# cts198859/deeprl_network

Hardware: AMD Instinct MI355X
Metric: env-steps/sec (agents x envs x steps/s), full rollout + A2C update loop (higher is better)
Workload: dtype f32; 1 GPU; CACC catchup, 8 agents x 4096 replicas/GPU, ia2c_fp (config_ia2c_fp_catchup.ini), n_step 60; replicas_per_gpu=4096, global_replicas=4096, parallelism=dp1, hipgraph_rollout=True, hipgraph_update=True, gemm_autotune=True

## Files before the change

deeprl_network_amd/_lib.py:

```python
import ctypes as C
import os

import torch

_PKG = os.path.dirname(os.path.abspath(__file__))
LIB_PATH = os.path.join(_PKG, 'libnmarl_hip.so')

if not os.path.exists(LIB_PATH):
    raise ImportError(
        'deeprl_network_amd: %s not found. Build it with `python -m deeprl_network_amd.build` '
        '(hipcc --offload-arch=gfx950). There is no CPU fallback.' % LIB_PATH)

from . import build as _build

if _build.built_hash() != _build.source_hash():
    raise ImportError(
        'deeprl_network_amd: %s is stale (built from sources %s, current sources %s). Rebuild it with '
        '`python -m deeprl_network_amd.build`.' % (LIB_PATH, _build.built_hash(), _build.source_hash()))

LIB_PATH = os.environ.get('NMARL_LIB_AB') or LIB_PATH
lib = C.CDLL(LIB_PATH)

ABI_VERSION = 4

# ... 179 lines not shown
    'nmarl_lstm_bptt_dial': [C.POINTER(BpttDial), _p],
    'nmarl_fc_fwd': [_i64, _i32, _i32, _i32, _p, _i64, _i64, _p, _i64, _p, _i64, _i32, _p, _i64, _i64, _p],
    'nmarl_fc_fwd_multi': [_i64, _i32, _i32, C.POINTER(FcPart), _i32, _p, _i64, _i64, _p],
    'nmarl_dial_msg_adjoint': [_i64, _i32, _i32, _p, _i64, _p, _i64, _p, _i64, _p, _i64, _p, _i64, _p, _i64, _p, _p, _p, _i32,
                               _p, _i64, _p, _i64, _p, _i64, _p, _i64, _p, _i64, _p],
    'nmarl_dial_msg_adjoint_parts': [_i64],
    'nmarl_onehot_argmax_add': [_i64, _i32, _i32, _i32, _p, _i64, _p, _p, _i64, _i64, _p],
    'nmarl_fc_bwd_chunks': [_i64, _i32],
    'nmarl_fc_bwd': [_i64, _i32, _i32, _i32, _p, _i64, _i64, _p, _i64, _i64, _p, _i64, _i64, _i32, _p, _p, _i64, _p, _i64, _p],
    'nmarl_fc_bwd_pair': [_i64, _i32, _p, _p, _i64, _i64, _p, _i64, _p, _i64, _i64, _i32, _p, _p, _p],
    'nmarl_fc_bwd_gather': [_i64, _i32, _i32, _i32, _p, _i32, _p, _i64, _i64, _p, _i64, _i64, _p, _i64, _i64, _i32, _p, _p, _i64, _p, _i64, _p],
    'nmarl_heads_loss': [_i64, _i32, _i32, _i32, _p, _i64, _p, _i64, _p, _i64, _p, _p, _p, _p, _f32, _f32, _p, _p, _p, _p, _p, _i64, _p, _i64, _p,
                         _i64, _p],
    'nmarl_thin_linear_bwd': [_i64, _i32, _i32, _i32, _p, _i64, _p, _i64, _p, _i64, _p, _i64, _p, _p, _i64, _p, _i64, _p, _i64, _p],
    'nmarl_nbr_action_value_fwd': [_i64, _i32, _i32, _i32, _p, _p, _p, _i64, _p, _i32, _p],
    'nmarl_nbr_action_value_bwd': [_i64, _i32, _i32, _i32, _p, _p, _p, _p, _p, _i64, _p],
    'nmarl_bias_act': [_i64, _i32, _i32, _p, _i64, _p, _i64, _i32, _p, _i64, _i64, _p],
    'nmarl_lstm_cell_bwd': [_i64, _i32, _i32, _p, _i64, _p, _i64, _p, _i64, _p, _p, _i64, _p, _i64, _p, _i64, _p, _i64, _p, _i64, _p],
    'nmarl_a2c_loss_chunks': [_i64, _i32],
    'nmarl_a2c_loss_fwd': [_i64, _i32, _i32, _p, _i64, _i64, _p, _p, _p, _p, _f32, _f32, _p, _p, _p],
    'nmarl_a2c_loss_bwd': [_i64, _i32, _i32, _p, _i64, _i64, _p, _p, _p, _p, _f32, _f32, _p, _p, _p, _p],
    'nmarl_sample_actions': [_i64, _i32, _i32, _p, _p, _i32, _u64, _i64, _i64, _p, _p, _p],
    'nmarl_nstep_return': [_i64, _i32, _i32, _p, _p, _p, _p, C.c_double, C.c_double, _p, _p, _p, _p],
    'nmarl_rmsprop_tf_clip': [_i32, _i64, _p, _p, _p, _p, _p, _f32, _f32, _f32, _f32, _f32, _p, _p],
    'nmarl_rmsprop_tf_clip_guarded': [_i32, _i64, _p, _p, _p, _p, _p, _f32, _f32, _f32, _f32, _f32, _p, _p, _p],
    'nmarl_handoff_capacity': [_i32, _i32],
    'nmarl_test_handoff_fault': [_i32],
    'nmarl_batch_epilogue': [C.POINTER(BatchEpilogue), _p],
    'nmarl_timestamp': [_p, _p],
    'nmarl_timestamp_rate_khz': [],
    'nmarl_copy_multi': [_i32, C.POINTER(_p), C.POINTER(_p), C.POINTER(_i64), _p, _p],
}

for _name, _args in SIGNATURES.items():
    _fn = getattr(lib, _name)
    _fn.argtypes = _args
    _fn.restype = C.c_int

if lib.nmarl_abi_version() != ABI_VERSION:
    raise ImportError('libnmarl_hip.so ABI %d != binding ABI %d: rebuild' %
                      (lib.nmarl_abi_version(), ABI_VERSION))


class NmarlError(RuntimeError):
    pass

# ... 24 lines not shown
```

deeprl_network_amd/agents/models.py:

```python
import logging
import os

import numpy as np
import torch

from .. import ops
from .policies import (ConsensusPolicy, DIALMultiAgentPolicy, FPPolicy, IC3MultiAgentPolicy, LstmPolicy,
                       NCMultiAgentPolicy)
from .utils import Scheduler

F32 = torch.float32


class IA2C:

    policy_cls = LstmPolicy
    per_agent_optimizer = True
    uses_fingerprint = False

    def __init__(self, n_s_ls, n_a_ls, neighbor_mask, distance_mask, coop_gamma, total_step, model_config,
                 seed=0, num_envs=1, device='cuda', dist_group=None, n_feat=None, n_feat_ls=None, obs_order=None):
        self.name = getattr(self, 'name', 'ia2c')
        self._init_algo(n_s_ls, n_a_ls, neighbor_mask, distance_mask, coop_gamma, total_step, seed,
                        model_config, num_envs, device, dist_group, n_feat, n_feat_ls, obs_order)
# ... 250 lines not shown
                os.environ.get('NMARL_MSG_CARRY', '1') == '0':
            return None
        if self._carry_buf is None:
            self._carry_buf = torch.zeros(self.n_agent, self.E, self.n_lstm, dtype=F32, device=self.device)
        d = dict(carry_in=self._carry_buf if (t > 0 and self._carry_holds == t) else None,
                 carry_out=self._carry_buf if t < self.n_step else None)
        mm = getattr(p, '_extra_full', {}).get('MM')
        if mm is not None and t + 1 < self.n_step and p.msg_kind == ops.MSG_MEAN_ADD:
            d['mean_next'] = mm[:, t + 1]
        self._carry_holds = t + 1 if t < self.n_step else -1
        return d

    S_bits = None

    def _relu_bits(self, t):
        if os.environ.get('NMARL_FC_BWD_PAIR', '1') == '0' or not getattr(self.policy, 'enc_writes_bits', False):
            return None
        if self.S_bits is None:
            self.S_bits = torch.zeros(self.n_agent, self.n_step, self.E, 4, dtype=torch.int32, device=self.device)
        p = self.policy
        p._bits_steps = 1 if t == 0 else p._bits_steps + 1
        return self.S_bits[:, t]

    def record(self, reward, done_post):
        t = self.t
        self.buf_r[t].copy_(self._norm_reward(reward))
        self.buf_done_post[t].copy_(done_post)
        self.t = t + 1

    def _norm_reward(self, r):
        if self.reward_norm > 0:
            r = r / self.reward_norm
        if self.reward_clip > 0:
            r = torch.clamp(r, -self.reward_clip, self.reward_clip)
        return r

    def load_rewards(self, raw_rewards):
        if self.reward_norm > 0:
            torch.div(raw_rewards, self.reward_norm, out=self.buf_r)
        else:
            torch.mul(raw_rewards, 1.0, out=self.buf_r)
        if self.reward_clip > 0:
            self.buf_r.clamp_(-self.reward_clip, self.reward_clip)
        self.t = self.n_step

    def bootstrap(self, done, action_scratch, mode=ops.SAMPLE_PHILOX, u=None, seed=0, env_id_base=0,
                  step=0, step_dev=None, done_is_zero=False, pre_encoded=False):
        assert self.t == self.n_step
        p = self.policy
        ob = None
        if pre_encoded:
            enc = self.encode_target(self.n_step)
        elif self.save_acts and p.enc_in_kernel(self.E, self.compact_obs):
            enc, ob = (self.encode_target(self.n_step) if p.coupled else None), dict(x=self.buf_x[self.n_step], fp=self.fp)
        elif self.save_acts and p.encodes_in_step(self.E, self.compact_obs):
            enc, ob = self.encode_target(self.n_step), self.buf_x[self.n_step]
        else:
            enc = p.encode(self.buf_x[self.n_step], self.fp)
        if self.save_acts and p.pv_one_launch(self.E):
            T = self.n_step
# ... 61 lines not shown
        per_agent = policy_loss + value_loss + entropy_loss
        self.last_loss = (policy_loss.detach(), value_loss.detach(), entropy_loss.detach(), per_agent.detach())
        return per_agent.sum()

    def update(self, R_end, rotate=True):
        lr = self.update_begin()
        self.update_grads(R_end)
        self.update_reduce()
        self.update_apply(lr, rotate=rotate)
        self.update_end()

    def update_begin(self):
        assert self.t == self.n_step, 'update() needs a full n_step batch (got %d)' % self.t
        self.cur_lr = self.lr_scheduler.get(self.n_step)
        return self.cur_lr

    @property
    def handoff_guarded(self):
        return bool(self.policy.coupled) and self.device.type == 'cuda'

    def update_grads(self, R_end):
        alpha = self.coop_gamma if self.coop_gamma >= 0 else -1.0
        T = self.n_step
        if self.save_acts and self.policy.pv_one_launch(self.E):
            with torch.no_grad():
                vn = self.buf_vn.view(self.n_agent, T * self.E)
                ops.nbr_action_value(self.buf_act.view(T * self.E, self.n_agent), self.policy.nbr_idx,
                                     self.policy.params['v_w'][:, self.n_lstm:], self.n_a, out=vn, accumulate=True)
                self.buf_v.copy_(self.buf_vn.permute(1, 0, 2))
        ops.nstep_return(self.buf_r, self.buf_v, self.buf_done_post, R_end.contiguous(), self.gamma, alpha,
                         self.dist_dev, self.R, self.Adv)
        ps = self.policy.params
        ps.begin_backward()
        FP = self.buf_fp[:T].permute(1, 0, 2, 3).reshape(self.n_agent, T * self.E, self.n_a)
        X = self.buf_x[:T]
        if self.save_acts:
            kw = {}
            if self.S_bits is not None and self.policy._bits_steps == T:
                kw['S_bits'] = self.S_bits
            Hs = self.policy.unroll_saved(X, FP, self.S_buf, self.G_buf, self.H_all, self.C_all,
                                          self.buf_done_pre, masked_steps=self.masked_steps, S_ext=self.S_ext, **kw)
        else:
            Hs = self.policy.unroll(X, FP, self.buf_done_pre, self.h_bw, self.c_bw, masked_steps=self.masked_steps)
        if not self._loss_backward_fused(Hs):
            loss = self._loss(Hs)
            loss.backward()
        ps.end_backward()
        if ps.mask is not None:
            ps.grad.mul_(ps.mask)
        if self._status_on_wire:
            ps.grad_tail.copy_(ops.handoff_status(self.device)[:1])

    @property
    def _status_on_wire(self):
# ... 14 lines not shown
            st = ops.handoff_status(self.device)[:1]
            torch.maximum(st, (ps.grad_tail != 0).to(torch.int32), out=st)
        if self.per_agent_optimizer:
            ops.rmsprop_tf_clip(ps.flat, ps.grad, ps.ms, ps.scratch, lr, self.rmsp_alpha, self.rmsp_epsilon,
                                self.max_grad_norm, scale, self.grad_norm, lr_dev=lr_dev, guard=guard)
        else:
            n = self.n_agent * ps.P
            ops.rmsprop_tf_clip(ps.flat.view(1, n), ps.grad.view(1, n), ps.ms.view(1, n), ps.scratch, lr,
                                self.rmsp_alpha, self.rmsp_epsilon, self.max_grad_norm, scale, self.grad_norm,
                                lr_dev=lr_dev, guard=guard)
        self._after_apply()
        if rotate:
            T = self.n_step
            self.h_bw.copy_(self.h_fw)
            self.c_bw.copy_(self.c_fw)
            self.buf_x[0].copy_(self.buf_x[T])
            self.buf_fp[0].copy_(self.buf_fp[T])

    def _after_apply(self):
        """Hook behind the optimiser step (ConseNet: the consensus averaging)."""

    def update_end(self):
        self.t = 0
        self.policy._enc_was_saved = False
        self.policy._bits_steps = 0
        self.policy._mm_was_saved = False

    def _obs_to_slab(self, obs):
        p = self.policy
        F, A = self.n_feat, self.n_a
        slab = np.zeros((1, self.n_agent, p.n_obs), dtype=np.float32)
        fp = None
        if not self._is_ma2c() and self.uses_fingerprint_obs():
            fp = np.zeros((self.n_agent, 1, p.n_na), dtype=np.float32)
        for i in range(self.n_agent):
            o = np.asarray(obs[i], dtype=np.float32)
            slab[0, i, :p.n_own[i]] = o[:p.n_own[i]]
            if self._is_ma2c():
                continue
            pos = p.n_own[i]
            for j in p.obs_order[i]:
                k = p.nbrs[i].index(j)
                slab[0, i, (k + 1) * F:(k + 1) * F + p.n_own[j]] = o[pos:pos + p.n_own[j]]
                pos += p.n_own[j]
            if fp is not None:
                for j in p.obs_order[i]:
# ... 176 lines not shown
```

deeprl_network_amd/csrc/a2c.hip:

```cpp
#include "common.h"

namespace {

__device__ __forceinline__ float sigmoidf_(float x) { return 1.0f / (1.0f + expf(-x)); }

struct CellStrides { int64_t z, z2, bias, c_prev, gates, c_new, h_new, dh, dh2, dc, dz, dc_prev; };

__global__ __launch_bounds__(256) void lstm_cell_fwd_kernel(
    const int64_t E, const int N, const int H, const CellStrides st, const float* __restrict__ z,
    const float* __restrict__ z2, const float* __restrict__ bias, const float* __restrict__ c_prev,
    const float* __restrict__ done, float* __restrict__ gates, float* __restrict__ c_new,
    float* __restrict__ h_new) {
    const int H4 = H >> 2;
    const int64_t total = (int64_t)N * E * H4;
    for (int64_t idx = (int64_t)blockIdx.x * blockDim.x + threadIdx.x; idx < total; idx += (int64_t)gridDim.x * blockDim.x) {
        const int64_t row = idx / H4;
        const int j = (int)(idx - row * H4) * 4;
        const int64_t n = row / E;
        const int64_t e = row - n * E;
        const float* zr = z + n * st.z + e * 4 * H;
        const float* b = bias + n * st.bias;
        float4 zi = *reinterpret_cast<const float4*>(zr + j), zf = *reinterpret_cast<const float4*>(zr + H + j);
        float4 zo = *reinterpret_cast<const float4*>(zr + 2 * H + j), zu = *reinterpret_cast<const float4*>(zr + 3 * H + j);
        if (z2 != nullptr) {
// ... 104 lines not shown
        } else {
            float uu;
            if (mode == 0) {
                uu = u[idx];
            } else {
                const Philox4 r = philox4x32_10((uint32_t)(env_id_base + e), (uint32_t)(n >> 2), (uint32_t)step,
                                                NMARL_STREAM_ACTION, (uint32_t)seed, (uint32_t)(seed >> 32));
                const uint32_t w = (n & 3) == 0 ? r.x : (n & 3) == 1 ? r.y : (n & 3) == 2 ? r.z : r.w;
                uu = u01_from_bits(w);
            }
            double tot = 0.0;
            for (int k = 0; k < A; ++k) tot += (double)p[k];
            double cum = 0.0;
            for (int k = 0; k < A; ++k) {
                cum += (double)p[k];
                if (cum / tot <= (double)uu) a = k + 1;
            }
            if (a > A - 1) a = A - 1;
        }
        action[idx] = (uint8_t)a;
    }
}

__global__ __launch_bounds__(256) void nstep_kernel(
    const int64_t E, const int N, const int T, const float* __restrict__ r, const float* __restrict__ v,
    const uint8_t* __restrict__ done_post, const float* __restrict__ R_end, const double gamma,
    const double alpha, const int32_t* __restrict__ dist, float* __restrict__ R_out, float* __restrict__ adv_out) {
    __shared__ double s_w[64 * 64];
    const bool spatial = alpha >= 0.0;
    if (spatial) {
        for (int p = threadIdx.x; p < N * N; p += blockDim.x) s_w[p] = dist[p] < 0 ? 0.0 : pow(alpha, (double)dist[p]);
        __syncthreads();
    }
    const int64_t total = (int64_t)N * E;
    for (int64_t idx = (int64_t)blockIdx.x * blockDim.x + threadIdx.x; idx < total; idx += (int64_t)gridDim.x * blockDim.x) {
        const int n = (int)(idx / E);
        const int64_t e = idx - (int64_t)n * E;
        double R = (double)R_end[idx];
        if (!spatial) {
            constexpr int U = 10;
            for (int t0 = T - 1; t0 >= 0; t0 -= U) {
                float rr[U], vv[U];
                uint8_t dd[U];
#pragma unroll
                for (int k = 0; k < U; ++k) {
                    const int t = t0 - k >= 0 ? t0 - k : 0;
                    dd[k] = done_post[(int64_t)t * E + e];
                    rr[k] = r[(int64_t)t * E + e];
                    vv[k] = v[((int64_t)t * N + n) * E + e];
                }
#pragma unroll
                for (int k = 0; k < U; ++k) {
                    const int t = t0 - k;
                    if (t < 0) break;
                    R = (double)rr[k] + gamma * R * (1.0 - (double)dd[k]);
                    const int64_t o = ((int64_t)n * T + t) * E + e;
                    R_out[o] = (float)R;
                    adv_out[o] = (float)(R - (double)vv[k]);
                }
            }
            continue;
        }
        for (int t = T - 1; t >= 0; --t) {
            const double keep = 1.0 - (double)done_post[(int64_t)t * E + e];
            if (!spatial) {
                R = (double)r[(int64_t)t * E + e] + gamma * R * keep;
            } else {
                R = gamma * R * keep;
                const float* rt = r + ((int64_t)t * E + e) * N;
                double add = 0.0;
                for (int j = 0; j < N; ++j) add += s_w[n * N + j] * (double)rt[j];
                R += add;
            }
            const int64_t o = ((int64_t)n * T + t) * E + e;
            R_out[o] = (float)R;
            adv_out[o] = (float)(R - (double)v[((int64_t)t * N + n) * E + e]);
        }
    }
}

struct EpilogueArgs {
    int64_t E;
    int32_t N, H, A, F, T, T_env;
    const float* g;
    const uint8_t* done;
    double *ep_sum, *ep_sq, *ep_len, *fin;
    float *h_fw, *c_fw, *h_bw, *c_bw;
    const float *fp_T, *fp_uniform, *x_T;
    float *fp_0, *x_0, *done_pre;
    const int32_t* skip_if;
};

constexpr int EPI_BLOCK = 256;
constexpr int EPI_MAX_BLOCKS = 1024;

__global__ __launch_bounds__(EPI_BLOCK) void epilogue_stats_kernel(const EpilogueArgs a, double* __restrict__ partial) {
    if (a.skip_if && *a.skip_if != 0) return;
    double f0 = 0.0, f1 = 0.0, f2 = 0.0, f3 = 0.0;
    for (int64_t e = (int64_t)blockIdx.x * EPI_BLOCK + threadIdx.x; e < a.E; e += (int64_t)gridDim.x * EPI_BLOCK) {
        double s = 0.0, q = 0.0;
// ... 256 lines not shown
    hipLaunchKernelGGL(bias_act_kernel, dim3(grid_x((int64_t)N * rows * W / 4)), dim3(256), 0,
                       static_cast<hipStream_t>(stream), rows, N, W, x, x_sn, bias, bias_sn, act, y, y_sn, y_row);
    return nmarl_check_launch();
}

extern "C" int nmarl_sample_actions(int64_t E, int32_t N, int32_t A, const float* pi, const float* u, int32_t mode,
                                    uint64_t seed, int64_t env_id_base, int64_t step, const int64_t* step_dev,
                                    uint8_t* action, void* stream) {
    if (E < 0 || N <= 0 || A <= 0 || A > 255 || mode < 0 || mode > 2 || (E > 0 && (!pi || !action))) return NMARL_EINVAL;
    if (mode == 0 && E > 0 && !u) return NMARL_EINVAL;
    if (E == 0) return NMARL_OK;
    hipLaunchKernelGGL(sample_kernel, dim3(grid_x(E * N)), dim3(256), 0, static_cast<hipStream_t>(stream), E, N, A, pi,
                       u, mode, seed, env_id_base, step, step_dev, action);
    return nmarl_check_launch();
}

extern "C" int nmarl_nstep_return(int64_t E, int32_t N, int32_t T, const float* r, const float* v,
                                  const uint8_t* done_post, const float* R_end, double gamma, double alpha,
                                  const int32_t* dist, float* R_out, float* adv_out, void* stream) {
    if (E < 0 || N <= 0 || N > 64 || T <= 0 || (E > 0 && (!r || !v || !done_post || !R_end || !R_out || !adv_out)))
        return NMARL_EINVAL;
    if (alpha >= 0.0 && !dist) return NMARL_EINVAL;
    if (E == 0) return NMARL_OK;
    hipLaunchKernelGGL(nstep_kernel, dim3(grid_x((int64_t)N * E)), dim3(256), 0, static_cast<hipStream_t>(stream), E, N,
                       T, r, v, done_post, R_end, gamma, alpha, dist, R_out, adv_out);
    return nmarl_check_launch();
}

extern "C" int nmarl_rmsprop_tf_clip_guarded(int32_t G, int64_t P, float* w, const float* g, float* ms, float* scratch,
                                             const float* lr_dev, float lr, float rho, float eps, float max_norm,
                                             float grad_scale, float* grad_norm_out, int32_t* status, void* stream) {
    if (G <= 0 || P <= 0 || !w || !g || !ms || !scratch || ((uintptr_t)status % 4)) return NMARL_EINVAL;
    hipStream_t s = static_cast<hipStream_t>(stream);
    hipLaunchKernelGGL(sumsq_kernel, dim3(SUMSQ_BLOCKS, G), dim3(256), 0, s, P, g, scratch);
    hipLaunchKernelGGL(rmsprop_kernel, dim3(grid_x(P, 1024), G), dim3(256), 0, s, P, w, g, ms, scratch, lr_dev, lr, rho,
                       eps, max_norm, grad_scale, grad_norm_out, status);
    return nmarl_check_launch();
}

extern "C" int nmarl_rmsprop_tf_clip(int32_t G, int64_t P, float* w, const float* g, float* ms, float* scratch,
                                     const float* lr_dev, float lr, float rho, float eps, float max_norm,
                                     float grad_scale, float* grad_norm_out, void* stream) {
    return nmarl_rmsprop_tf_clip_guarded(G, P, w, g, ms, scratch, lr_dev, lr, rho, eps, max_norm, grad_scale, grad_norm_out,
                                         nullptr, stream);
}

static int loss_chunks(int64_t rows, int N) {
    int64_t c = (rows * N + 4095) / 4096;
// ... 112 lines not shown
```

deeprl_network_amd/ops.py:

```python
import ctypes as C
import os

import numpy as np
import torch

from . import _lib
from ._lib import check, lib, ptr, stream

F32 = torch.float32


_handoff_status = {}
_handoff_off = [False]


def handoff_status(device):
    dev = torch.device(device)
    if dev.index is None:
        dev = torch.device('cuda', torch.cuda.current_device())
    if dev not in _handoff_status:
        _handoff_status[dev] = torch.zeros(4, dtype=torch.int32, device=dev)
    return _handoff_status[dev]


# ... 848 lines not shown
                                   ptr(dw), dw.stride(0), ptr(db), db.stride(0), stream()), 'nmarl_heads_loss')
        dwa = nbr_action_value_bwd(action, nbr_idx, dv, A)
        return dict(terms=terms, dh=dh, dy8=dy8, hw=w, pi_w=dw[:, :, :A], pi_b=db[:, :A],
                    v_w=torch.cat([dw[:, :, A:], dwa.unsqueeze(-1)], dim=1), v_b=db[:, A:])


def heads_supported(h, n_a, nbr_idx):
    return h.shape[2] == FC_J and n_a + 1 <= THIN_MAX_O and nbr_idx.shape[1] * n_a <= NBR_ACT_MAX_W


def heads(h, pi_w, pi_b, v_w, v_b, action, nbr_idx, n_a):
    return _Heads.apply(h, pi_w, pi_b, v_w, v_b, action, nbr_idx, n_a)


WGRAD_SPLIT = 16


def wgrad(a, g, out=None):
    N, rows, M = a.shape
    S = WGRAD_SPLIT
    if rows % S or rows < 64 * S or not a.is_contiguous() or not g.is_contiguous():
        r = torch.bmm(a.transpose(1, 2), g)
        return r if out is None else torch.mul(r, 1.0, out=out)
    part = torch.bmm(a.view(N * S, rows // S, M).transpose(1, 2), g.view(N * S, rows // S, g.shape[2]))
    part = part.view(N, S, M, g.shape[2])
    return part.sum(1) if out is None else torch.sum(part, dim=1, out=out)


class _Linear(torch.autograd.Function):

    @staticmethod
    def forward(ctx, x, w):
        ctx.save_for_backward(x, w)
        return torch.bmm(x, w)

    @staticmethod
    def backward(ctx, dy):
        x, w = ctx.saved_tensors
        dy = dy.contiguous()
        dx = torch.bmm(dy, w.transpose(1, 2)) if ctx.needs_input_grad[0] else None
        return dx, wgrad(x, dy)


def linear(x, w):
    return _Linear.apply(x, w)


def cell_bwd(gates, c_prev, c_new, done, dh, dc, dz, dc_prev, dh2=None):
    N, E, H4 = gates.shape
# ... 38 lines not shown


_pending_head_dy = {}


def head_dy_placeholder(dy8, hw, like):
    ph = torch.zeros(1, dtype=F32, device=like.device).expand(like.shape)
    _pending_head_dy[like.device] = (ph, dy8, hw)
    return ph


def take_head_dy(dHs):
    pend = _pending_head_dy.pop(dHs.device, None)
    if pend is None or dHs.data_ptr() != pend[0].data_ptr() or any(dHs.stride()):
        return None
    return pend[1], pend[2]


def head_dy_to_dh(dy8, hw, shape):
    O = hw.shape[2]
    return torch.bmm(dy8[:, :, :O], hw.transpose(1, 2)).view(shape)


def bptt_seq(G, Call, done, dHs, img, dZ, want_db=True, want_state_grad=False, head_dy=None):
    N, T, E, H4 = G.shape
    H = H4 // 4
    for x, w, what in ((G, H4, 'gates'), (dZ, H4, 'dz'), (Call, H, 'c_all')) + (((dHs, H, 'dh_ext'),) if head_dy is None else ()):
        if x.stride(3) != 1 or x.stride(2) != w:
            raise ValueError('bptt_seq: %s must have contiguous rows' % what)
    nblk = lib.nmarl_lstm_bptt_seq_blocks(E)
    part = torch.empty(N, nblk, H4, dtype=F32, device=G.device) if want_db else None
    dh0 = torch.empty(N, E, H, dtype=F32, device=G.device) if want_state_grad else None
    dc0 = torch.empty(N, E, H, dtype=F32, device=G.device) if want_state_grad else None
    if head_dy is None:
        dh, dy = (ptr(dHs, F32, strided=True), dHs.stride(0), dHs.stride(1)), (None, 0, 0, None, 0, 0)
    else:
        dy8, hw = head_dy
        if dy8.shape != (N, T * E, 8) or not dy8.is_contiguous() or hw.shape[:2] != (N, H) or not hw.is_contiguous():
            raise ValueError('bptt_seq: head_dy = (dy8 [N,T*E,8], hw [N,64,O]) contiguous')
        dh, dy = (None, 0, 0), (ptr(dy8, F32), dy8.stride(0), E * 8, ptr(hw, F32), hw.stride(0), hw.shape[2])
    check(lib.nmarl_lstm_bptt_seq(T, E, N, H, ptr(G, F32, strided=True), G.stride(0), G.stride(1), ptr(Call, F32, strided=True),
                                  Call.stride(0), Call.stride(1), ptr(done, F32), *dh, *dy, ptr(img, F32), img.stride(0),
                                  ptr(dZ, F32, strided=True), dZ.stride(0), dZ.stride(1), ptr(part), 0 if part is None else part.stride(0),
                                  *_pn(dh0), *_pn(dc0), stream()), 'nmarl_lstm_bptt_seq')
    return (part.sum(dim=1) if want_db else None), dh0, dc0


COUPLED_NC, COUPLED_IC3 = 1, 2
COUPLED_DIAL = 3


def dial_adjoint_supported(m_max, H, rev):
    return H == FUSED_H and m_max <= 4 and rev is not None and rev['r_max'] <= 4


def dial_adjoint_images(w_msg, mfc_w):
    N, K, H = w_msg.shape
    wt = w_msg.reshape(N, K // H, H, H).transpose(2, 3).reshape(N, K, H).contiguous()
    return lstm_msg_wimage(wt), lstm_msg_wimage(mfc_w.transpose(1, 2).contiguous())


def dial_adjoint_bias_parts(N, E, device):
    parts = lib.nmarl_dial_msg_adjoint_parts(E)
    return torch.zeros(N, parts, FUSED_H, dtype=F32, device=device), torch.zeros(N, parts, FUSED_H, dtype=F32, device=device)


def dial_msg_adjoint(ds, hm, msg, dhd, w_msg, mfc_w, nbr_idx, imgs, rev, d1, d2, dh, bias_parts=None):
# ... 355 lines not shown
                                                            ctx.needs_input_grad[0])
        return ds, dwx, dwh, db, dh_rec, dc, None, None, None


def _lstm_seq_x_backward(G, Hall, Call, s, wx, wh, done, masked, dHs, need_ds, want_state_grad=True, s_ext=None):
    N, T, E, H4 = G.shape
    H = H4 // 4
    head_dy = take_head_dy(dHs)
    one_launch = bptt_supported(H) and wh.stride(2) == 1 and wh.stride(1) == H4 and E <= BPTT_SEQ_MAX_E
    if head_dy is not None and not one_launch:
        dHs, head_dy = head_dy_to_dh(*head_dy, dHs.shape), None
    if head_dy is None:
        dHs = dHs.contiguous()
    keep = (1.0 - done)
    KX = s.shape[3]
    ext = (s_ext is not None and len(masked) < T and s_ext.shape == (N, T + 1, E, KX) and s_ext.is_contiguous() and Hall.is_contiguous()
           and s.data_ptr() == s_ext.data_ptr() and ((T + 1) * E) % WGRAD_SPLIT == 0)
    if ext:
        dZe = torch.empty(N, T + 1, E, H4, dtype=F32, device=G.device)
        dZe[:, T].zero_()
        dZ = dZe[:, :T]
    else:
        dZ = torch.empty_like(G)
    db = None
    if one_launch:
        db, dh_rec, dc = bptt_seq(G, Call, done, dHs, lstm_bptt_wimage(None, wh), dZ, want_state_grad=want_state_grad, head_dy=head_dy)
    else:
        dh_rec = None
        dc = torch.zeros(N, E, H, dtype=F32, device=G.device)
        dc_next = torch.empty_like(dc)
        wh_t = wh.transpose(1, 2)
        for t in range(T - 1, -1, -1):
            cell_bwd(G[:, t], Call[:, t], Call[:, t + 1], done[t], dHs[:, t], dc, dZ[:, t], dc_next, dh2=dh_rec)
            dc, dc_next = dc_next, dc
            dh_rec = torch.bmm(dZ[:, t], wh_t)
            if t in masked:
                dh_rec = dh_rec * keep[t].view(1, E, 1)
    dZf = dZ.reshape(N, T * E, H4)
    if ext:
        with torch.no_grad():
            for t in masked:
                Hall[:, t].mul_(keep[t].view(1, E, 1))
        dZx = dZe.view(N, (T + 1) * E, H4)
        dwh = wgrad(Hall.view(N, (T + 1) * E, H), dZx)
        dwx = wgrad(s_ext.view(N, (T + 1) * E, KX), dZx)
    else:
        if len(masked) == T:
            Hprev = (Hall[:, :T] * keep.view(1, T, E, 1)).reshape(N, T * E, H)
        else:
            Hprev = Hall[:, :T].clone()
            for t in masked:
                Hprev[:, t].mul_(keep[t].view(1, E, 1))
            Hprev = Hprev.view(N, T * E, H)
        dwh = wgrad(Hprev, dZf)
        dwx = wgrad(s.reshape(N, T * E, KX), dZf)
    if db is None:
        db = dZf.sum(dim=1)
    ds = torch.bmm(dZf, wx.transpose(1, 2)).view(N, T, E, KX) if need_ds else None
    return ds, dwx, dwh, db, dh_rec, dc


class _LstmSequenceSaved(torch.autograd.Function):

    @staticmethod
    def forward(ctx, s, wx, wh, b, G, Hall, Call, done, masked_steps, s_ext):
        T = G.shape[1]
        ctx.save_for_backward(G, Hall, Call, s, wx, wh, done)
        ctx.masked = set(range(T)) if masked_steps is None else set(masked_steps)
# ... 59 lines not shown
        check(lib.nmarl_a2c_loss_bwd(rows, N, A, ptr(logits, F32, strided=True), logits.stride(0), logits.stride(1), ptr(v, F32),
                                     ptr(action, torch.uint8), ptr(adv, F32), ptr(R, F32), ctx.coefs[0], ctx.coefs[1],
                                     ptr(gn, F32), ptr(dlogits), ptr(dv), stream()), 'nmarl_a2c_loss_bwd')
        return dlogits, dv, None, None, None, None, None


def a2c_loss_supported(n_a):
    return n_a <= A2C_LOSS_MAX_A


def a2c_loss(logits, v, action, adv, R, v_coef, e_coef):
    return _A2CLoss.apply(logits, v, action, adv, R, float(v_coef), float(e_coef))


def nstep_return(r, v, done_post, R_end, gamma, alpha, dist=None, R_out=None, adv_out=None):
    T, N, E = v.shape
    if R_out is None:
        R_out = torch.empty(N, T, E, dtype=F32, device=v.device)
    if adv_out is None:
        adv_out = torch.empty(N, T, E, dtype=F32, device=v.device)
    check(lib.nmarl_nstep_return(E, N, T, ptr(r, F32), ptr(v, F32), ptr(done_post, torch.uint8), ptr(R_end, F32),
                                 float(gamma), float(alpha), ptr(dist, torch.int32), ptr(R_out), ptr(adv_out),
                                 stream()), 'nmarl_nstep_return')
    return R_out, adv_out


def rmsprop_tf_clip(w, g, ms, scratch, lr, rho, eps, max_norm, grad_scale=1.0, norm_out=None, lr_dev=None, guard=False):
    G, P = w.shape
    check(lib.nmarl_rmsprop_tf_clip_guarded(G, P, ptr(w, F32), ptr(g, F32), ptr(ms, F32), ptr(scratch, F32),
                                            ptr(lr_dev, F32), float(lr), float(rho), float(eps), float(max_norm),
                                            float(grad_scale), ptr(norm_out, F32),
                                            ptr(handoff_status(w.device), torch.int32) if (guard and w.is_cuda) else None, stream()),
          'nmarl_rmsprop_tf_clip')


_epilogue_scratch = {}


def batch_epilogue(g, done, ep_sum, ep_sq, ep_len, fin, T_env, h_fw, c_fw, h_bw, c_bw, fp_T, fp_0, fp_uniform, x_T, x_0, done_pre,
                   skip_if=None):
    T, E = g.shape
    N, _, H = h_fw.shape
    a = _lib.BatchEpilogue()
    a.E, a.N, a.H, a.A, a.F, a.T, a.T_env = E, N, H, fp_T.shape[2], x_T.shape[2], T, int(T_env)
    a.g, a.done = ptr(g, F32), ptr(done, torch.uint8)
    a.ep_sum, a.ep_sq, a.ep_len, a.fin = (ptr(t, torch.float64) for t in (ep_sum, ep_sq, ep_len, fin))
# ... 41 lines not shown
```

include/nmarl.h:

```cpp
#ifndef NMARL_H
#define NMARL_H

#include <stdint.h>

#ifdef __cplusplus
extern "C" {
#endif

#define NMARL_OK 0
#define NMARL_EINVAL (-1)
#define NMARL_EHIP (-2)

#define NMARL_CACC_N 8
#define NMARL_CACC_NF 5
#define NMARL_CACC_OBS 15

int nmarl_abi_version(void);
const char* nmarl_source_hash(void);


typedef struct nmarl_cacc_params {
    float dt;
    float h_min;
    float h_star;
// ... 315 lines not shown
                     const float* b, int64_t b_sn, const float* va, const uint8_t* action, const float* adv, const float* R,
                     float v_coef, float e_coef, float* partial, float* loss_out, float* dy8, float* dv, float* dh,
                     int64_t dh_sn, float* dw, int64_t dw_sn, float* db, int64_t db_sn, void* stream);

int nmarl_nbr_action_value_fwd(int64_t rows, int32_t N, int32_t A, int32_t m_max, const int32_t* nbr_idx,
                               const uint8_t* action, const float* w, int64_t w_sn, float* va, int32_t accumulate,
                               void* stream);
int nmarl_nbr_action_value_bwd(int64_t rows, int32_t N, int32_t A, int32_t m_max, const int32_t* nbr_idx,
                               const uint8_t* action, const float* dv, float* partial, float* dw, int64_t dw_sn,
                               void* stream);
int nmarl_sample_actions(int64_t E, int32_t N, int32_t A, const float* pi, const float* u, int32_t mode,
                         uint64_t seed, int64_t env_id_base, int64_t step, const int64_t* step_dev,
                         uint8_t* action, void* stream);
int nmarl_a2c_loss_chunks(int64_t rows, int32_t N);
int nmarl_a2c_loss_fwd(int64_t rows, int32_t N, int32_t A, const float* logits, int64_t l_sn, int64_t l_row,
                       const float* v, const uint8_t* action, const float* adv, const float* R, float v_coef,
                       float e_coef, float* partial, float* loss_out, void* stream);
int nmarl_a2c_loss_bwd(int64_t rows, int32_t N, int32_t A, const float* logits, int64_t l_sn, int64_t l_row,
                       const float* v, const uint8_t* action, const float* adv, const float* R, float v_coef,
                       float e_coef, const float* g_up, float* dlogits, float* dv, void* stream);
int nmarl_nstep_return(int64_t E, int32_t N, int32_t T, const float* r, const float* v,
                       const uint8_t* done_post, const float* R_end, double gamma, double alpha,
                       const int32_t* dist, float* R_out, float* adv_out, void* stream);
int nmarl_handoff_capacity(int32_t which, int32_t K);
int nmarl_test_handoff_fault(int32_t nth);
int nmarl_rmsprop_tf_clip_guarded(int32_t G, int64_t P, float* w, const float* g, float* ms, float* scratch,
                                  const float* lr_dev, float lr, float rho, float eps, float max_norm, float grad_scale,
                                  float* grad_norm_out, int32_t* status, void* stream);
int nmarl_rmsprop_tf_clip(int32_t G, int64_t P, float* w, const float* g, float* ms, float* scratch,
                          const float* lr_dev, float lr, float rho, float eps, float max_norm,
                          float grad_scale, float* grad_norm_out, void* stream);

typedef struct nmarl_batch_epilogue {
    int64_t E;
    int32_t N, H, A, F, T, T_env;
    const float* g;
    const uint8_t* done;
    double *ep_sum, *ep_sq, *ep_len, *fin;
    float *h_fw, *c_fw, *h_bw, *c_bw;
    const float *fp_T, *fp_uniform, *x_T;
    float *fp_0, *x_0, *done_pre;
    double* scratch;
    const int32_t* skip_if;
} nmarl_batch_epilogue_t;
#define NMARL_EPILOGUE_SCRATCH 4096
int nmarl_batch_epilogue(const nmarl_batch_epilogue_t* p, void* stream);
// ... 13 lines not shown
```

Baseline: 245.7 million env-steps/s.

## Fuse reward normalization and value transpose into n-step return; batch wgrad slab sums

The n-step return kernel now normalizes and clips raw rewards itself and reads values through strides, writing the normalized rewards and transposed values as side outputs. This removes the separate div/clamp and permute-copy launches. The three split-K partial reductions in the LSTM weight-gradient path (dwh, dwx, db) are also replaced by one batched vectorized slab-sum kernel instead of three torch.sum calls. These changes cut launch count and memory passes in the update. They add new kernel paths and stateful deferral of reward normalization (_r_raw) that must stay consistent with later readers of buf_r.

```diff
diff --git a/deeprl_network_amd/_lib.py b/deeprl_network_amd/_lib.py
--- a/deeprl_network_amd/_lib.py
+++ b/deeprl_network_amd/_lib.py
@@ -225,6 +225,8 @@
     'nmarl_a2c_loss_bwd': [_i64, _i32, _i32, _p, _i64, _i64, _p, _p, _p, _p, _f32, _f32, _p, _p, _p, _p],
     'nmarl_sample_actions': [_i64, _i32, _i32, _p, _p, _i32, _u64, _i64, _i64, _p, _p, _p],
     'nmarl_nstep_return': [_i64, _i32, _i32, _p, _p, _p, _p, C.c_double, C.c_double, _p, _p, _p, _p],
+    'nmarl_nstep_return_norm': [_i64, _i32, _i32, _p, _f32, _f32, _p, _p, _i64, _i64, _p, _p, _p, C.c_double, C.c_double, _p, _p, _p, _p],
+    'nmarl_slab_sum': [_i32, _i32, _p, _p, _p, _p, _p, _p, _p],
     'nmarl_rmsprop_tf_clip': [_i32, _i64, _p, _p, _p, _p, _p, _f32, _f32, _f32, _f32, _f32, _p, _p],
     'nmarl_rmsprop_tf_clip_guarded': [_i32, _i64, _p, _p, _p, _p, _p, _f32, _f32, _f32, _f32, _f32, _p, _p, _p],
     'nmarl_handoff_capacity': [_i32, _i32],
diff --git a/deeprl_network_amd/agents/models.py b/deeprl_network_amd/agents/models.py
--- a/deeprl_network_amd/agents/models.py
+++ b/deeprl_network_amd/agents/models.py
@@ -296,8 +296,11 @@
         p._bits_steps = 1 if t == 0 else p._bits_steps + 1
         return self.S_bits[:, t]
 
+    _r_raw = None
+
     def record(self, reward, done_post):
         t = self.t
+        self._r_raw = None
         self.buf_r[t].copy_(self._norm_reward(reward))
         self.buf_done_post[t].copy_(done_post)
         self.t = t + 1
@@ -310,6 +313,11 @@
         return r
 
     def load_rewards(self, raw_rewards):
+        if raw_rewards.is_cuda and raw_rewards.shape == self.buf_r.shape and raw_rewards.is_contiguous() and \
+                raw_rewards.data_ptr() != self.buf_r.data_ptr():
+            self._r_raw = raw_rewards
+            self.t = self.n_step
+            return
         if self.reward_norm > 0:
             torch.div(raw_rewards, self.reward_norm, out=self.buf_r)
         else:
@@ -417,14 +425,23 @@
     def update_grads(self, R_end):
         alpha = self.coop_gamma if self.coop_gamma >= 0 else -1.0
         T = self.n_step
-        if self.save_acts and self.policy.pv_one_launch(self.E):
+        agent_major = self.save_acts and self.policy.pv_one_launch(self.E)
+        if agent_major:
             with torch.no_grad():
                 vn = self.buf_vn.view(self.n_agent, T * self.E)
                 ops.nbr_action_value(self.buf_act.view(T * self.E, self.n_agent), self.policy.nbr_idx,
                                      self.policy.params['v_w'][:, self.n_lstm:], self.n_a, out=vn, accumulate=True)
+        if self._r_raw is not None or (agent_major and self.buf_r.is_cuda):
+            raw = self._r_raw is not None
+            ops.nstep_return_norm(self._r_raw if raw else self.buf_r, self.reward_norm if raw else 0.0, self.reward_clip if raw else 0.0,
+                                  self.buf_r if raw else None, self.buf_vn.permute(1, 0, 2) if agent_major else self.buf_v,
+                                  self.buf_v if agent_major else None, self.buf_done_post, R_end.contiguous(), self.gamma, alpha,
+                                  self.dist_dev, self.R, self.Adv)
+        else:
+            if agent_major:
                 self.buf_v.copy_(self.buf_vn.permute(1, 0, 2))
-        ops.nstep_return(self.buf_r, self.buf_v, self.buf_done_post, R_end.contiguous(), self.gamma, alpha,
-                         self.dist_dev, self.R, self.Adv)
+            ops.nstep_return(self.buf_r, self.buf_v, self.buf_done_post, R_end.contiguous(), self.gamma, alpha,
+                             self.dist_dev, self.R, self.Adv)
         ps = self.policy.params
         ps.begin_backward()
         FP = self.buf_fp[:T].permute(1, 0, 2, 3).reshape(self.n_agent, T * self.E, self.n_a)
@@ -485,6 +502,7 @@
 
     def update_end(self):
         self.t = 0
+        self._r_raw = None
         self.policy._enc_was_saved = False
         self.policy._bits_steps = 0
         self.policy._mm_was_saved = False
diff --git a/deeprl_network_amd/csrc/a2c.hip b/deeprl_network_amd/csrc/a2c.hip
--- a/deeprl_network_amd/csrc/a2c.hip
+++ b/deeprl_network_amd/csrc/a2c.hip
@@ -150,10 +150,19 @@
     }
 }
 
+template <bool NORM>
 __global__ __launch_bounds__(256) void nstep_kernel(
     const int64_t E, const int N, const int T, const float* __restrict__ r, const float* __restrict__ v,
     const uint8_t* __restrict__ done_post, const float* __restrict__ R_end, const double gamma,
-    const double alpha, const int32_t* __restrict__ dist, float* __restrict__ R_out, float* __restrict__ adv_out) {
+    const double alpha, const int32_t* __restrict__ dist, float* __restrict__ R_out, float* __restrict__ adv_out,
+    const float r_scale, const float r_clip, float* __restrict__ r_norm_out, const int64_t v_st, const int64_t v_sn,
+    float* __restrict__ v_out) {
+    auto norm = [&](float x) {
+        if (!NORM) return x;
+        x = x * r_scale;
+        if (r_clip > 0.0f) x = x < -r_clip ? -r_clip : (x > r_clip ? r_clip : x);
+        return x;
+    };
     __shared__ double s_w[64 * 64];
     const bool spatial = alpha >= 0.0;
     if (spatial) {
@@ -174,13 +183,17 @@
                 for (int k = 0; k < U; ++k) {
                     const int t = t0 - k >= 0 ? t0 - k : 0;
                     dd[k] = done_post[(int64_t)t * E + e];
-                    rr[k] = r[(int64_t)t * E + e];
-                    vv[k] = v[((int64_t)t * N + n) * E + e];
+                    rr[k] = norm(r[(int64_t)t * E + e]);
+                    vv[k] = v[(int64_t)t * v_st + (int64_t)n * v_sn + e];
                 }
 #pragma unroll
                 for (int k = 0; k < U; ++k) {
                     const int t = t0 - k;
                     if (t < 0) break;
+                    if (NORM) {
+                        if (n == 0 && r_norm_out) r_norm_out[(int64_t)t * E + e] = rr[k];
+                        if (v_out) v_out[((int64_t)t * N + n) * E + e] = vv[k];
+                    }
                     R = (double)rr[k] + gamma * R * (1.0 - (double)dd[k]);
                     const int64_t o = ((int64_t)n * T + t) * E + e;
                     R_out[o] = (float)R;
@@ -192,18 +205,69 @@
         for (int t = T - 1; t >= 0; --t) {
             const double keep = 1.0 - (double)done_post[(int64_t)t * E + e];
             if (!spatial) {
-                R = (double)r[(int64_t)t * E + e] + gamma * R * keep;
+                R = (double)norm(r[(int64_t)t * E + e]) + gamma * R * keep;
             } else {
                 R = gamma * R * keep;
                 const float* rt = r + ((int64_t)t * E + e) * N;
                 double add = 0.0;
-                for (int j = 0; j < N; ++j) add += s_w[n * N + j] * (double)rt[j];
+                for (int j = 0; j < N; ++j) {
+                    const float rj = norm(rt[j]);
+                    if (NORM && n == 0 && r_norm_out) r_norm_out[((int64_t)t * E + e) * N + j] = rj;
+                    add += s_w[n * N + j] * (double)rj;
+                }
                 R += add;
             }
             const int64_t o = ((int64_t)n * T + t) * E + e;
+            const float vt = v[(int64_t)t * v_st + (int64_t)n * v_sn + e];
+            if (NORM && v_out) v_out[((int64_t)t * N + n) * E + e] = vt;
             R_out[o] = (float)R;
-            adv_out[o] = (float)(R - (double)v[((int64_t)t * N + n) * E + e]);
-        }
+            adv_out[o] = (float)(R - (double)vt);
+        }
+    }
+}
+
+constexpr int SLAB_JOBS = 3;
+struct SlabSumJob {
+    const float* part;
+    float* out;
+    int64_t part_sn, out_sn, C;
+    int S;
+};
+struct SlabSumArgs { SlabSumJob job[SLAB_JOBS]; };
+
+__global__ __launch_bounds__(256) void slab_sum_kernel(const SlabSumArgs a) {
+    const SlabSumJob j = a.job[blockIdx.z];
+    const int n = blockIdx.y;
+    const int64_t C4 = j.C >> 2;
+    const float4* __restrict__ p = reinterpret_cast<const float4*>(j.part + (int64_t)n * j.part_sn);
+    float4* __restrict__ o = reinterpret_cast<float4*>(j.out + (int64_t)n * j.out_sn);
+    for (int64_t i = (int64_t)blockIdx.x * blockDim.x + threadIdx.x; i < C4; i += (int64_t)gridDim.x * blockDim.x) {
+        float4 acc[4];
+#pragma unroll
+        for (int u = 0; u < 4; ++u) acc[u] = make_float4(0.0f, 0.0f, 0.0f, 0.0f);
+        int s = 0;
+        for (; s + 3 < j.S; s += 4) {
+            float4 v[4];
+#pragma unroll
+            for (int u = 0; u < 4; ++u) v[u] = p[(int64_t)(s + u) * C4 + i];
+#pragma unroll
+            for (int u = 0; u < 4; ++u) {
+                acc[u].x += v[u].x; acc[u].y += v[u].y; acc[u].z += v[u].z; acc[u].w += v[u].w;
+            }
+        }
+#pragma unroll
+        for (int u = 0; u < 3; ++u) {
+            if (s + u < j.S) {
+                const float4 v = p[(int64_t)(s + u) * C4 + i];
+                acc[u].x += v.x; acc[u].y += v.y; acc[u].z += v.z; acc[u].w += v.w;
+            }
+        }
+        float4 r;
+        r.x = ((acc[0].x + acc[1].x) + acc[2].x) + acc[3].x;
+        r.y = ((acc[0].y + acc[1].y) + acc[2].y) + acc[3].y;
+        r.z = ((acc[0].z + acc[1].z) + acc[2].z) + acc[3].z;
+        r.w = ((acc[0].w + acc[1].w) + acc[2].w) + acc[3].w;
+        o[i] = r;
     }
 }
 
@@ -506,8 +570,47 @@
         return NMARL_EINVAL;
     if (alpha >= 0.0 && !dist) return NMARL_EINVAL;
     if (E == 0) return NMARL_OK;
-    hipLaunchKernelGGL(nstep_kernel, dim3(grid_x((int64_t)N * E)), dim3(256), 0, static_cast<hipStream_t>(stream), E, N,
-                       T, r, v, done_post, R_end, gamma, alpha, dist, R_out, adv_out);
+    hipLaunchKernelGGL(nstep_kernel<false>, dim3(grid_x((int64_t)N * E)), dim3(256), 0, static_cast<hipStream_t>(stream), E, N,
+                       T, r, v, done_post, R_end, gamma, alpha, dist, R_out, adv_out, 1.0f, 0.0f, (float*)nullptr, (int64_t)N * E, E,
+                       (float*)nullptr);
+    return nmarl_check_launch();
+}
+
+extern "C" int nmarl_nstep_return_norm(int64_t E, int32_t N, int32_t T, const float* r_raw, float r_scale, float r_clip,
+                                       float* r_norm_out, const float* v, int64_t v_st, int64_t v_sn, float* v_out,
+                                       const uint8_t* done_post, const float* R_end, double gamma, double alpha,
+                                       const int32_t* dist, float* R_out, float* adv_out, void* stream) {
+    if (E < 0 || N <= 0 || N > 64 || T <= 0 || (E > 0 && (!r_raw || !v || !done_post || !R_end || !R_out || !adv_out)))
+        return NMARL_EINVAL;
+    if (alpha >= 0.0 && !dist) return NMARL_EINVAL;
+    if (v_st < E || v_sn < E || !((v_st >= (int64_t)N * v_sn) || (v_sn >= (int64_t)T * v_st))) return NMARL_EINVAL;
+    if (v_out == v || r_norm_out == r_raw || !(r_scale == r_scale)) return NMARL_EINVAL;
+    if (E == 0) return NMARL_OK;
+    hipLaunchKernelGGL(nstep_kernel<true>, dim3(grid_x((int64_t)N * E)), dim3(256), 0, static_cast<hipStream_t>(stream), E, N,
+                       T, r_raw, v, done_post, R_end, gamma, alpha, dist, R_out, adv_out, r_scale, r_clip, r_norm_out, v_st, v_sn,
+                       v_out);
+    return nmarl_check_launch();
+}
+
+extern "C" int nmarl_slab_sum(int32_t N, int32_t n_jobs, const float* const* part, const int64_t* part_sn, const int32_t* S,
+                              const int64_t* C, float* const* out, const int64_t* out_sn, void* stream) {
+    if (N <= 0 || n_jobs <= 0 || n_jobs > SLAB_JOBS || !part || !part_sn || !S || !C || !out || !out_sn) return NMARL_EINVAL;
+    SlabSumArgs a;
+    int64_t cmax = 0;
+    for (int k = 0; k < n_jobs; ++k) {
+        if (!part[k] || !out[k] || S[k] <= 0 || C[k] <= 0 || (C[k] & 3) || part_sn[k] < (int64_t)S[k] * C[k] || out_sn[k] < C[k] ||
+            (part_sn[k] & 3) || (out_sn[k] & 3) || ((uintptr_t)part[k] & 15) || ((uintptr_t)out[k] & 15))
+            return NMARL_EINVAL;
+        a.job[k].part = part[k];
+        a.job[k].out = out[k];
+        a.job[k].part_sn = part_sn[k];
+        a.job[k].out_sn = out_sn[k];
+        a.job[k].C = C[k];
+        a.job[k].S = S[k];
+        cmax = C[k] > cmax ? C[k] : cmax;
+    }
+    for (int k = n_jobs; k < SLAB_JOBS; ++k) a.job[k] = a.job[0];
+    hipLaunchKernelGGL(slab_sum_kernel, dim3(grid_x(cmax >> 2, 256), N, n_jobs), dim3(256), 0, static_cast<hipStream_t>(stream), a);
     return nmarl_check_launch();
 }
 
diff --git a/deeprl_network_amd/ops.py b/deeprl_network_amd/ops.py
--- a/deeprl_network_amd/ops.py
+++ b/deeprl_network_amd/ops.py
@@ -894,9 +894,51 @@
     if rows % S or rows < 64 * S or not a.is_contiguous() or not g.is_contiguous():
         r = torch.bmm(a.transpose(1, 2), g)
         return r if out is None else torch.mul(r, 1.0, out=out)
+    part = wgrad_parts(a, g)
+    if not a.is_cuda:
+        return part.sum(1) if out is None else torch.sum(part, dim=1, out=out)
+    if out is None:
+        out = torch.empty(N, M, g.shape[2], dtype=F32, device=a.device)
+    slab_sum([(part, out)])
+    return out
+
+
+def wgrad_splits(a, g):
+    rows, S = a.shape[1], WGRAD_SPLIT
+    return not (rows % S or rows < 64 * S or not a.is_contiguous() or not g.is_contiguous())
+
+
+def wgrad_parts(a, g):
+    N, rows, M = a.shape
+    S = WGRAD_SPLIT
     part = torch.bmm(a.view(N * S, rows // S, M).transpose(1, 2), g.view(N * S, rows // S, g.shape[2]))
-    part = part.view(N, S, M, g.shape[2])
-    return part.sum(1) if out is None else torch.sum(part, dim=1, out=out)
+    return part.view(N, S, M, g.shape[2])
+
+
+SLAB_JOBS = 3
+
+
+def slab_sum(jobs):
+    jobs = list(jobs)
+    for i in range(0, len(jobs), SLAB_JOBS):
+        chunk = jobs[i:i + SLAB_JOBS]
+        n = len(chunk)
+        N = chunk[0][0].shape[0]
+        cs = []
+        for part, out in chunk:
+            c = part[0, 0].numel()
+            if part.shape[0] != N or out.shape[0] != N or out[0].numel() != c or not part.is_contiguous() or not out[0].is_contiguous() \
+                    or part.dtype != F32 or out.dtype != F32:
+                raise _lib.NmarlError('slab_sum: part [N,S,...] contiguous f32, out [N,...] f32 with contiguous per-agent panels (got %s -> %s)'
+                                      % (tuple(part.shape), tuple(out.shape)))
+            cs.append(c)
+        pp = (C.c_void_p * n)(*[ptr(part, F32) for part, _ in chunk])
+        po = (C.c_void_p * n)(*[ptr(out, F32, strided=True) for _, out in chunk])
+        psn = (C.c_int64 * n)(*[part.stride(0) if N > 1 else part[0].numel() for part, _ in chunk])
+        osn = (C.c_int64 * n)(*[out.stride(0) if N > 1 else c for (_, out), c in zip(chunk, cs)])
+        ss = (C.c_int32 * n)(*[part.shape[1] for part, _ in chunk])
+        cc = (C.c_int64 * n)(*cs)
+        check(lib.nmarl_slab_sum(N, n, pp, psn, ss, cc, po, osn, stream()), 'nmarl_slab_sum')
 
 
 class _Linear(torch.autograd.Function):
@@ -981,7 +1023,7 @@
     return torch.bmm(dy8[:, :, :O], hw.transpose(1, 2)).view(shape)
 
 
-def bptt_seq(G, Call, done, dHs, img, dZ, want_db=True, want_state_grad=False, head_dy=None):
+def bptt_seq(G, Call, done, dHs, img, dZ, want_db=True, want_state_grad=False, head_dy=None, db_parts=False):
     N, T, E, H4 = G.shape
     H = H4 // 4
     for x, w, what in ((G, H4, 'gates'), (dZ, H4, 'dz'), (Call, H, 'c_all')) + (((dHs, H, 'dh_ext'),) if head_dy is None else ()):
@@ -1002,6 +1044,8 @@
                                   Call.stride(0), Call.stride(1), ptr(done, F32), *dh, *dy, ptr(img, F32), img.stride(0),
                                   ptr(dZ, F32, strided=True), dZ.stride(0), dZ.stride(1), ptr(part), 0 if part is None else part.stride(0),
                                   *_pn(dh0), *_pn(dc0), stream()), 'nmarl_lstm_bptt_seq')
+    if want_db and db_parts:
+        return part, dh0, dc0
     return (part.sum(dim=1) if want_db else None), dh0, dc0
 
 
@@ -1403,9 +1447,11 @@
         dZ = dZe[:, :T]
     else:
         dZ = torch.empty_like(G)
-    db = None
+    db, one_sum = None, False
     if one_launch:
-        db, dh_rec, dc = bptt_seq(G, Call, done, dHs, lstm_bptt_wimage(None, wh), dZ, want_state_grad=want_state_grad, head_dy=head_dy)
+        one_sum = ext and G.is_cuda and wgrad_splits(Hall.view(N, (T + 1) * E, H), dZe) and wgrad_splits(s_ext.view(N, (T + 1) * E, KX), dZe)
+        db, dh_rec, dc = bptt_seq(G, Call, done, dHs, lstm_bptt_wimage(None, wh), dZ, want_state_grad=want_state_grad, head_dy=head_dy,
+                                  db_parts=one_sum)
     else:
         dh_rec = None
         dc = torch.zeros(N, E, H, dtype=F32, device=G.device)
@@ -1423,8 +1469,14 @@
             for t in masked:
                 Hall[:, t].mul_(keep[t].view(1, E, 1))
         dZx = dZe.view(N, (T + 1) * E, H4)
-        dwh = wgrad(Hall.view(N, (T + 1) * E, H), dZx)
-        dwx = wgrad(s_ext.view(N, (T + 1) * E, KX), dZx)
+        if one_launch and one_sum:
+            ph, px, pb = wgrad_parts(Hall.view(N, (T + 1) * E, H), dZx), wgrad_parts(s_ext.view(N, (T + 1) * E, KX), dZx), db
+            dwh, dwx, db = (torch.empty(N, H, H4, dtype=F32, device=G.device), torch.empty(N, KX, H4, dtype=F32, device=G.device),
+                            torch.empty(N, H4, dtype=F32, device=G.device))
+            slab_sum([(ph, dwh), (px, dwx), (pb, db)])
+        else:
+            dwh = wgrad(Hall.view(N, (T + 1) * E, H), dZx)
+            dwx = wgrad(s_ext.view(N, (T + 1) * E, KX), dZx)
     else:
         if len(masked) == T:
             Hprev = (Hall[:, :T] * keep.view(1, T, E, 1)).reshape(N, T * E, H)
@@ -1530,6 +1582,28 @@
     check(lib.nmarl_nstep_return(E, N, T, ptr(r, F32), ptr(v, F32), ptr(done_post, torch.uint8), ptr(R_end, F32),
                                  float(gamma), float(alpha), ptr(dist, torch.int32), ptr(R_out), ptr(adv_out),
                                  stream()), 'nmarl_nstep_return')
+    return R_out, adv_out
+
+
+def reward_scale(reward_norm):
+    return float(np.float32(1.0) / np.float32(reward_norm)) if reward_norm > 0 else 1.0
+
+
+def nstep_return_norm(r_raw, reward_norm, reward_clip, r_out, v, v_out, done_post, R_end, gamma, alpha, dist=None, R_out=None,
+                      adv_out=None):
+    T, N, E = v.shape
+    if v.stride(2) != 1 and E > 1:
+        raise _lib.NmarlError('nstep_return_norm: v needs unit stride over the replicas')
+    if R_out is None:
+        R_out = torch.empty(N, T, E, dtype=F32, device=v.device)
+    if adv_out is None:
+        adv_out = torch.empty(N, T, E, dtype=F32, device=v.device)
+    if r_out is not None and r_out.shape != r_raw.shape:
+        raise _lib.NmarlError('nstep_return_norm: r_out must have the shape of r_raw')
+    check(lib.nmarl_nstep_return_norm(E, N, T, ptr(r_raw, F32), reward_scale(reward_norm), float(reward_clip) if reward_clip > 0 else 0.0,
+                                      ptr(r_out, F32), ptr(v, F32, strided=True), v.stride(0), v.stride(1), ptr(v_out, F32),
+                                      ptr(done_post, torch.uint8), ptr(R_end, F32), float(gamma), float(alpha), ptr(dist, torch.int32),
+                                      ptr(R_out), ptr(adv_out), stream()), 'nmarl_nstep_return_norm')
     return R_out, adv_out
 
 
diff --git a/include/nmarl.h b/include/nmarl.h
--- a/include/nmarl.h
+++ b/include/nmarl.h
@@ -361,6 +361,12 @@
 int nmarl_nstep_return(int64_t E, int32_t N, int32_t T, const float* r, const float* v,
                        const uint8_t* done_post, const float* R_end, double gamma, double alpha,
                        const int32_t* dist, float* R_out, float* adv_out, void* stream);
+int nmarl_nstep_return_norm(int64_t E, int32_t N, int32_t T, const float* r_raw, float r_scale, float r_clip,
+                            float* r_norm_out, const float* v, int64_t v_st, int64_t v_sn, float* v_out,
+                            const uint8_t* done_post, const float* R_end, double gamma, double alpha,
+                            const int32_t* dist, float* R_out, float* adv_out, void* stream);
+int nmarl_slab_sum(int32_t N, int32_t n_jobs, const float* const* part, const int64_t* part_sn, const int32_t* S,
+                   const int64_t* C, float* const* out, const int64_t* out_sn, void* stream);
 int nmarl_handoff_capacity(int32_t which, int32_t K);
 int nmarl_test_handoff_fault(int32_t nth);
 int nmarl_rmsprop_tf_clip_guarded(int32_t G, int64_t P, float* w, const float* g, float* ms, float* scratch,
```

Result: slower. 242.5 million env-steps/s (-1.3%).
